# CristianSimion5/vk-raytracing-engine

Measured on AMD Instinct MI355X. Metric: Mrays/s, higher is better.
Workload: dtype f32

## Files before the change

include/vkrt.h:

```cpp
#ifndef VKRT_H
#define VKRT_H

#include <stdint.h>
#include "vkrt_host_device.h"

#ifdef __cplusplus
extern "C" {
#endif

#define VKRT_ABI_VERSION 4

enum vkrt_status {
  VKRT_OK = 0,
  VKRT_ERR_INVALID_ARGUMENT = 1,
  VKRT_ERR_NO_DEVICE = 2,
  VKRT_ERR_HIP = 3,
  VKRT_ERR_OUT_OF_MEMORY = 4,
  VKRT_ERR_NOT_BUILT = 5,
  VKRT_ERR_UNSUPPORTED = 6
};

typedef struct vkrt_scene vkrt_scene;

typedef struct vkrt_prim_mesh {
// ... 86 lines not shown
  uint32_t build_flags;
  float    sah_cost;
  float    build_ms;
  uint64_t node_bytes;
  uint64_t triangle_bytes;
  uint32_t reference_count;
  uint32_t reserved;
} vkrt_accel_info;

int         vkrt_abi_version(void);
const char* vkrt_last_error(void);
int         vkrt_device_count(void);

int  vkrt_scene_create(const vkrt_scene_desc* desc, int device, vkrt_scene** out);
void vkrt_scene_destroy(vkrt_scene* scene);

enum vkrt_option {
  VKRT_OPT_MODE            = 1,
  VKRT_OPT_BVH_LAYOUT      = 2,
  VKRT_OPT_WF_SUBFRAMES    = 3,
  VKRT_OPT_WF_TRAV_BLOCK   = 4,
  VKRT_OPT_WF_SHARE        = 5,
  VKRT_OPT_TRI_THRESHOLD   = 6,
  VKRT_OPT_WF_SHARE_PERIOD = 7,
  VKRT_OPT_WF_SHARE_FLAGS  = 8,
  VKRT_OPT_GBUFFER_MIPS    = 9,
  VKRT_OPT_WATERTIGHT      = 10,
  VKRT_OPT_SKIP_DEAD_SHADOW_RAYS = 11,
  VKRT_OPT_ANYHIT_DISSOLVE = 12,
  VKRT_OPT_WF_FRAMES_IN_FLIGHT = 13,
  VKRT_OPT_SPLIT_BUDGET    = 14,
  VKRT_OPT_LAST            = 14,
  VKRT_OPT_WF_SAMPLE_SYNC  = 15,
  VKRT_INFO_ANYHIT_ORDER   = 100,
  VKRT_INFO_SPLIT_BUDGET   = 101
};
int vkrt_scene_set_option(vkrt_scene* scene, int option, int value);
int vkrt_scene_get_option(const vkrt_scene* scene, int option, int* value);

int vkrt_accel_build(vkrt_scene* scene, uint32_t build_flags, void* hip_stream);
int vkrt_accel_get_info(const vkrt_scene* scene, vkrt_accel_info* out);

int vkrt_scene_update_nodes(vkrt_scene* scene, uint32_t first, uint32_t count, const vkrt_node* nodes, void* hip_stream);
int vkrt_accel_refit(vkrt_scene* scene, void* hip_stream);

enum vkrt_memory { VKRT_MEMORY_HOST = 0, VKRT_MEMORY_DEVICE = 1 };
typedef struct vkrt_vertex_update {
  uint32_t struct_size;
  uint32_t first, count;
  uint32_t memory;
  const float* positions;
  const float* normals;
  const float* tangents;
  const float* texcoords0;
} vkrt_vertex_update;
int vkrt_scene_update_vertices(vkrt_scene* scene, const vkrt_vertex_update* update, void* hip_stream);

typedef struct vkrt_ray {
  float origin[3];    float tmin;
  float direction[3]; float tmax;
} vkrt_ray;
typedef struct vkrt_hit {
  float   t, u, v;
  int32_t instance;
  int32_t primitive;
  int32_t prim_mesh;
// ... 146 lines not shown
```

vk-raytracing-engine_amd/abi.py:

```python
import ctypes as C

c_f = C.c_float
c_i = C.c_int32
c_u = C.c_uint32
c_u64 = C.c_uint64


class Mat4(C.Structure):
    _fields_ = [("m", c_f * 16)]


class GlobalUniforms(C.Structure):
    _fields_ = [("viewProj", Mat4), ("viewInverse", Mat4), ("projInverse", Mat4)]


class PushConstantRay(C.Structure):
    _fields_ = [
        ("clearColor", c_f * 4),
        ("frame", c_i),
        ("lightsCount", c_i),
        ("samples", c_i),
        ("depth", c_i),
        ("useShadows", c_i),
        ("useAO", c_i),
# ... 170 lines not shown
                ("tangents", C.c_void_p), ("texcoords0", C.c_void_p)]


assert C.sizeof(VertexUpdate) == 48
assert C.sizeof(Ray) == 32
assert C.sizeof(Hit) == 32
assert C.sizeof(Surface) == 128
assert C.sizeof(InstanceVisibility) == 4
assert C.sizeof(QueryOpts) == 16

assert C.sizeof(GlobalUniforms) == 192
assert C.sizeof(PushConstantRay) == 44
assert C.sizeof(PrimMeshInfo) == 12
assert C.sizeof(GltfPBRMaterial) == 52
assert C.sizeof(GltfLight) == 32
assert C.sizeof(PrimMesh) == 20
assert C.sizeof(Node) == 68

VKRT_OK, VKRT_ERR_INVALID_ARGUMENT, VKRT_ERR_NO_DEVICE, VKRT_ERR_HIP, VKRT_ERR_OUT_OF_MEMORY, VKRT_ERR_NOT_BUILT, VKRT_ERR_UNSUPPORTED = range(7)
VKRT_BUILD_LBVH_GPU = 0x1
VKRT_BUILD_SAH_HOST = 0x2
VKRT_BUILD_PLOC_GPU = 0x4
VKRT_TRACE_SEED_INDEX_ROW_MAJOR = 0x1
VKRT_TRACE_COUNT_TRAVERSAL = 0x2
VKRT_TRACE_TIME_KERNELS = 0x4
VKRT_TRACE_SAME_SEED_EVERY_FRAME = 0x8
VKRT_ABI_VERSION = 4
VKRT_OPT_MODE, VKRT_OPT_BVH_LAYOUT, VKRT_OPT_WF_SUBFRAMES, VKRT_OPT_WF_TRAV_BLOCK = 1, 2, 3, 4
VKRT_OPT_WF_SHARE, VKRT_OPT_TRI_THRESHOLD, VKRT_OPT_WF_SHARE_PERIOD, VKRT_OPT_WF_SHARE_FLAGS = 5, 6, 7, 8
VKRT_OPT_GBUFFER_MIPS = 9
VKRT_OPT_WATERTIGHT, VKRT_OPT_SKIP_DEAD_SHADOW_RAYS, VKRT_OPT_ANYHIT_DISSOLVE = 10, 11, 12
VKRT_OPT_WF_FRAMES_IN_FLIGHT, VKRT_OPT_SPLIT_BUDGET = 13, 14
VKRT_OPT_WF_SAMPLE_SYNC = 15
VKRT_INFO_ANYHIT_ORDER = 100
VKRT_INFO_SPLIT_BUDGET = 101
VKRT_INSTANCE_FACING_CULL_DISABLE, VKRT_INSTANCE_FLIP_FACING = 0x1, 0x2
VKRT_RAY_OPAQUE, VKRT_RAY_CULL_BACK_FACING, VKRT_RAY_CULL_FRONT_FACING = 0x1, 0x10, 0x20
VKRT_MEMORY_HOST, VKRT_MEMORY_DEVICE = 0, 1
VKRT_SURFACE_GEOMETRY, VKRT_SURFACE_MATERIAL = 0x1, 0x2
VKRT_MULTIHIT_MAX = 16

VKRT_SYMBOLS = [
    "vkrt_abi_version",
    "vkrt_last_error",
    "vkrt_device_count",
    "vkrt_scene_create",
    "vkrt_scene_destroy",
    "vkrt_scene_set_option",
    "vkrt_scene_get_option",
    "vkrt_reserve",
    "vkrt_reserve_frames",
    "vkrt_accel_build",
    "vkrt_accel_get_info",
    "vkrt_scene_update_nodes",
    "vkrt_accel_refit",
    "vkrt_scene_update_vertices",
    "vkrt_intersect",
    "vkrt_occluded",
    "vkrt_scene_set_instance_visibility",
    "vkrt_scene_get_instance_visibility",
    "vkrt_intersect_ex",
    "vkrt_occluded_ex",
    "vkrt_intersect_multi",
    "vkrt_closest_point",
    "vkrt_hit_surface",
    "vkrt_shard_rows",
# ... 122 lines not shown
```

vk-raytracing-engine_amd/csrc/device_scene.h:

```cpp
#pragma once
#include <hip/hip_runtime.h>
#include <stdint.h>
#include "../../include/vkrt_host_device.h"
#include "device_math.h"

struct DevInstance
{
  float o2w[12];
  float w2o[9];
  int32_t primMesh;
  uint32_t vis;
  int32_t pad;
};
static_assert(sizeof(DevInstance) == 96, "DevInstance");
#define VKRT_VIS_CULL_DISABLE 0x100u
#define VKRT_VIS_FLIP 0x200u
#define VKRT_VIS_MIRRORED 0x10000u

#define VKRT_VERTEX_QUADS 3
#define VKRT_VERTEX_BYTES 48u
struct DevTexRef
{
  uint32_t offset;
  uint32_t wh;
// ... 66 lines not shown
  unsigned long long* faults;
};
struct DevQueryScene : DevScene
{
  const uint2* nodeMasks;
  uint32_t cullMask;
  uint32_t rayFlags;
};
struct DevSurfaceScene : DevScene
{
  const uint4* primMeshes;
  uint32_t instanceCount;
};

#define VKRT_TRAV_FAULT(sc) atomicAdd((sc).faults, 1ull)

#ifndef VKRT_W8_MAX_POSTPONED
#define VKRT_W8_MAX_POSTPONED 8
#endif
#ifndef VKRT_W8_POSTPONE_ROOM
#define VKRT_W8_POSTPONE_ROOM 0
#endif

#define VKRT_COUNTER_SLOTS 64
struct DevCounters
{
  unsigned long long v[VKRT_COUNTER_SLOTS][VKRT_COUNTER_STRIDE];
};

#define VKRT_TRACE_PUBLIC_FLAGS 0xFu
#define VKRT_FLAG_SKIP_DEAD_SHADOW 0x100u
#define VKRT_FLAG_STORE_STAGED 0x200u
#define VKRT_FLAG_SAMPLE_SYNC 0x400u

struct TraceParams
{
  DevScene sc;
  PushConstantRay pc;
  float viewInverse[16];
  float projInverse[16];
  uint32_t seed;
  uint32_t flags;
  uint32_t fullW, fullH;
  uint32_t stripRows, shardCount, shardIndex;
  uint32_t localRows;
  uint32_t tilesX, tileCount;
  uint32_t tileFirst;
  float* image;
  unsigned int* workCounter;
  DevCounters* counters;
};

struct WfBuffers
{
  unsigned* ctrl;
  float4* planes;
  float4* stage;
  uint32_t capacity;
  uint32_t groups;
  float4* sampleState;
};
```

vk-raytracing-engine_amd/csrc/kernels.h:

```cpp
#pragma once
#include <hip/hip_runtime.h>
#include "device_scene.h"

hipError_t vkrt_launch_pathtrace(const TraceParams& P, unsigned gridBlocks, bool count, hipStream_t stream);
int        vkrt_pathtrace_block_size();
hipError_t vkrt_pathtrace_occupancy(size_t ldsBytes, int* blocksPerCU);
hipError_t vkrt_launch_trace_rays(const DevScene& sc, unsigned n, const float* o, const float* d, float tmin, float tmax, int anyHit,
                                  float* t, float* u, float* v, int* gid, hipStream_t stream);
hipError_t vkrt_launch_eval_math(int op, unsigned n, const float* a, const float* b, float* out, hipStream_t stream);

hipError_t vkrt_launch_query(const DevQueryScene& sc, const float4* rays, uint64_t n, uint32_t seed, bool filter, bool opaque, float4* hits, int* occ,
                             hipStream_t stream);
hipError_t vkrt_launch_query_multi(const DevQueryScene& sc, const float4* rays, uint64_t n, uint32_t seed, bool filter, bool opaque, uint32_t maxHits,
                                   float4* hits, int* counts, hipStream_t stream);
hipError_t vkrt_launch_closest_point(const DevQueryScene& sc, const float4* queries, uint64_t n, bool filter, float4* hits, unsigned long long* work,
                                     hipStream_t stream);
hipError_t vkrt_launch_node_masks(const DevScene& sc, uint32_t nodeCount, uint32_t instCount, uint32_t sweeps, uint2* masks, hipStream_t stream);
hipError_t vkrt_launch_hit_surface(const DevSurfaceScene& sc, const float4* hits, uint32_t n, bool material, float4* out, hipStream_t stream);

struct WfTiming
{
  hipEvent_t* events;
  int capacity;
  int used;
};
#define VKRT_WF_MAX_LANES 8
struct WfAsync
{
  hipStream_t streams[VKRT_WF_MAX_LANES];
  hipEvent_t fork, join[VKRT_WF_MAX_LANES];
  int count;
  hipEvent_t* pool;
  int poolSize;
};
inline int vkrt_wf_pool_events(int frames, int lanes) { return frames * lanes; }
size_t     vkrt_wf_state_bytes(uint32_t pathCapacity, int groups);
void       vkrt_wf_carve(void* base, uint32_t pathCapacity, int groups, WfBuffers* B);
struct WfOptions
{
  int subframes;
  int travBlock;
  int inFlight;
};
hipError_t vkrt_launch_wavefront(const TraceParams& P, const WfBuffers& B, const WfOptions& opt, int frames, uint32_t seedStep, bool count,
                                 hipStream_t stream, WfTiming* timing, const WfAsync* async);
void       vkrt_wf_launch_traverse(const TraceParams& P, const WfBuffers& B, int r, unsigned travBlock, bool count, dim3 tg, size_t tlds,
                                   hipStream_t stream);

struct HybridGi
{
  float4* color;
  float4* position;
  float4* normal;
  float2* rough;
  float4* accum;
  float4* nrdRadHitD;
  float* nrdViewZ;
};
hipError_t vkrt_launch_gbuffer(const TraceParams& P, const float clearColor[4], int lightsCount, const HybridGi& G, float* nrdNormRough,
                               const float* viewMatrix, hipStream_t stream);
hipError_t vkrt_launch_hybrid(const TraceParams& P, const HybridGi& G, uint2* giLater, hipStream_t stream);
hipError_t vkrt_launch_hybrid_gi(const TraceParams& P, const WfBuffers& B, const HybridGi& G, unsigned travBlock, hipStream_t stream);
uint2* vkrt_wf_hybrid_tmp(const WfBuffers& B);
hipError_t vkrt_launch_post(int rtMode, int viewAccumulated, int useGI, unsigned n, const float* mainImg, const float* rtImg, float* out,
                            hipStream_t stream);

struct DenoiseParams
{
  uint32_t W, H;
  const float4* color;
  const float4* position;
  const float4* normal;
  const float2* rough;
  const float* viewZ;
  const float4* radHitD;
  const float4* histColor;
  const float4* geomPrev;
  float4* geomCur;
  const float4* momPrev;
  float4* momCur;
// ... 25 lines not shown
```

vk-raytracing-engine_amd/csrc/vkrt_api.cpp:

```cpp
#include <hip/hip_runtime.h>

#include <algorithm>
#include <chrono>
#include <cmath>
#include <cstdarg>
#include <cstdio>
#include <cstdlib>
#include <cstring>
#include <initializer_list>
#include <string>
#include <vector>

#include "../../include/vkrt.h"
#include "bvh_host.h"
#include "dev_buffer.h"
#include "device_scene.h"
#include "kernels.h"
#include "wide_node.h"

#define VKRT_TRI_THRESHOLD_DEFAULT 32
#define VKRT_WF_SHARE_DEFAULT 16
#define VKRT_WF_SHARE_FLAGS_DEFAULT 25
#define VKRT_WF_FRAMES_IN_FLIGHT_DEFAULT 3
#define VKRT_SPLIT_BUDGET_DEFAULT -1
#define VKRT_WF_SAMPLE_SYNC_DEFAULT 1
#include "lbvh.h"
#include "refit.h"
#include "vertex_update.h"

namespace {

thread_local std::string g_lastError;

int fail(int code, const char* fmt, ...)
{
  char buf[512];
  va_list ap;
  va_start(ap, fmt);
  vsnprintf(buf, sizeof buf, fmt, ap);
  va_end(ap);
  g_lastError = buf;
  return code;
}

#define HIP_TRY(expr)                                                      \
  do                                                                       \
  {                                                                        \
    std::string m_;                                                        \
    if(const int rc_ = vkrt::hip_status((expr), #expr, m_); rc_ != VKRT_OK) \
      return fail(rc_, "%s", m_.c_str());                                  \
  } while(0)

}

struct vkrt_scene
{
  int device = 0;
  int cuCount = 256;
  std::vector<float> positions;
  std::vector<uint32_t> indices;
  std::vector<vkrt_prim_mesh> primMeshes;
  std::vector<vkrt_node> nodes;
  uint32_t lightCount = 0, materialCount = 0;
  std::vector<float> materialAlpha;
  std::vector<void*> allocs;
  DevScene dev{};
  vkrt::TreeBuffers accel;
  bool built = false;
  vkrt_accel_info info{};
  unsigned int* workCounter = nullptr;
  DevCounters* counters = nullptr;
  hipEvent_t evStart = nullptr, evStop = nullptr;
  bool timed = false;
  void* wfMem = nullptr;
  WfBuffers wf{};
  WfAsync wfAsync{};
  std::vector<hipEvent_t> wfEvents;
  WfTiming wfTiming{};
  bool wfTimed = false;
  int splitResolved = 0;
  int wfTimingRounds = 0;
  std::vector<hipEvent_t> wfPool;
  int opt[VKRT_OPT_WF_SAMPLE_SYNC + 1] = {0, 1, 1, 3, 64, VKRT_WF_SHARE_DEFAULT, VKRT_TRI_THRESHOLD_DEFAULT, 0, VKRT_WF_SHARE_FLAGS_DEFAULT, 1, 0, 0, 0,
                                          VKRT_WF_FRAMES_IN_FLIGHT_DEFAULT, VKRT_SPLIT_BUDGET_DEFAULT, VKRT_WF_SAMPLE_SYNC_DEFAULT};
  bool hasLargeTriangles = false;
  bool wavefront = true;
  bool stale = false;
  bool refitted = false;
  vkrt::RefitScratch refit;
  bool positionsOnDevice = false;
  vkrt::DevBuf vertexStage;
  size_t vertexStageBytes = 0;
  std::vector<vkrt_instance_visibility> vis;
  uint64_t masksPresent[4] = {0, 0, 0, 0};
  vkrt::DevBuf nodeMasks;
  const uint4* surfacePrimMeshes = nullptr;
};

namespace {

template <typename T>
int upload(vkrt_scene* s, const T* src, size_t count, const T** dst)
{
  void* p = nullptr;
  const size_t bytes = std::max<size_t>(count * sizeof(T), 16);
  HIP_TRY(hipMalloc(&p, bytes));
  s->allocs.push_back(p);
  if(count)
    HIP_TRY(hipMemcpy(p, src, count * sizeof(T), hipMemcpyHostToDevice));
  *dst = (const T*)p;
  return VKRT_OK;
}

int checkTransform(const vkrt_node& n, uint32_t i)
{
  for(int k = 0; k < 16; k++)
    if(!std::isfinite(n.worldMatrix[k]))
// ... 65 lines not shown
      const float flx = floorf(fu), fly = floorf(fv), ax = fu - flx, ay = fv - fly;
      auto cl = [](int v, int n) { return v < 0 ? 0 : (v >= n ? n - 1 : v); };
      const int x0 = cl((int)flx, (int)sw), x1 = cl((int)flx + 1, (int)sw), y0 = cl((int)fly, (int)sh), y1 = cl((int)fly + 1, (int)sh);
      const uint32_t p[4] = {src[(size_t)y0 * sw + x0], src[(size_t)y0 * sw + x1], src[(size_t)y1 * sw + x0], src[(size_t)y1 * sw + x1]};
      uint32_t out = 0;
      for(int c = 0; c < 4; c++)
      {
        const uint32_t base = (srgb && c < 3) ? 0u : 256u;
        const float t00 = lut512[base + ((p[0] >> (8 * c)) & 255u)], t10 = lut512[base + ((p[1] >> (8 * c)) & 255u)];
        const float t01 = lut512[base + ((p[2] >> (8 * c)) & 255u)], t11 = lut512[base + ((p[3] >> (8 * c)) & 255u)];
        float v = (t00 * (1.0f - ax) + t10 * ax) * (1.0f - ay) + (t01 * (1.0f - ax) + t11 * ax) * ay;
        if(srgb && c < 3) v = srgbEncode(v);
        v = v < 0.0f ? 0.0f : (v > 1.0f ? 1.0f : v);
        out |= (uint32_t)(v * 255.0f + 0.5f) << (8 * c);
      }
      dst[(size_t)y * dw + x] = out;
    }
}

bool useWavefront(const vkrt_scene* s) { return s->opt[VKRT_OPT_MODE] == 1; }

int clampOption(int option, int v)
{
  switch(option)
  {
    case VKRT_OPT_MODE: case VKRT_OPT_BVH_LAYOUT: return v ? 1 : 0;
    case VKRT_OPT_WF_SUBFRAMES: case VKRT_OPT_WF_FRAMES_IN_FLIGHT: return std::max(1, std::min(VKRT_WF_MAX_LANES, v));
    case VKRT_OPT_SPLIT_BUDGET: return std::max(-1, std::min(100, v));
    case VKRT_OPT_WF_TRAV_BLOCK: return v == 256 ? 256 : v == 128 ? 128 : 64;
    case VKRT_OPT_WF_SHARE: return std::max(0, std::min(64, v));
    case VKRT_OPT_TRI_THRESHOLD: return std::max(0, std::min(65, v));
    case VKRT_OPT_WF_SHARE_PERIOD: return std::max(0, std::min(255, v));
    case VKRT_OPT_WF_SHARE_FLAGS: return v & 31;
    case VKRT_OPT_GBUFFER_MIPS: case VKRT_OPT_WATERTIGHT: case VKRT_OPT_SKIP_DEAD_SHADOW_RAYS: case VKRT_OPT_ANYHIT_DISSOLVE: case VKRT_OPT_WF_SAMPLE_SYNC: return v ? 1 : 0;
  }
  return v;
}

void optionsFromEnvironment(vkrt_scene* s)
{
  const char* e;
  if((e = getenv("VKRT_MODE")) && !strcmp(e, "mega")) s->opt[VKRT_OPT_MODE] = 0;
  if((e = getenv("VKRT_BVH")) && !strcmp(e, "bvh2")) s->opt[VKRT_OPT_BVH_LAYOUT] = 0;
  const struct { const char* name; int option; } ints[] = {{"VKRT_WF_SUBFRAMES", VKRT_OPT_WF_SUBFRAMES}, {"VKRT_WF_TRAV_BLOCK", VKRT_OPT_WF_TRAV_BLOCK},
                                                          {"VKRT_WF_SHARE", VKRT_OPT_WF_SHARE}, {"VKRT_TRI_THRESHOLD", VKRT_OPT_TRI_THRESHOLD},
                                                          {"VKRT_WF_SHARE_PERIOD", VKRT_OPT_WF_SHARE_PERIOD}, {"VKRT_WF_SHARE_FLAGS", VKRT_OPT_WF_SHARE_FLAGS},
                                                          {"VKRT_GBUFFER_MIPS", VKRT_OPT_GBUFFER_MIPS}, {"VKRT_WATERTIGHT", VKRT_OPT_WATERTIGHT},
                                                          {"VKRT_SKIP_DEAD_SHADOW_RAYS", VKRT_OPT_SKIP_DEAD_SHADOW_RAYS},
                                                          {"VKRT_ANYHIT_DISSOLVE", VKRT_OPT_ANYHIT_DISSOLVE}, {"VKRT_WF_FRAMES_IN_FLIGHT", VKRT_OPT_WF_FRAMES_IN_FLIGHT},
                                                          {"VKRT_SPLIT_BUDGET", VKRT_OPT_SPLIT_BUDGET}, {"VKRT_WF_SAMPLE_SYNC", VKRT_OPT_WF_SAMPLE_SYNC}};
  for(const auto& k : ints)
    if((e = getenv(k.name)))
      s->opt[k.option] = clampOption(k.option, atoi(e));
}

void freeAccel(vkrt_scene* s)
{
  s->accel = vkrt::TreeBuffers{};
  s->nodeMasks = vkrt::DevBuf{};
  s->built = false;
  s->refit = vkrt::RefitScratch{};
  s->refitted = false;
  s->stale = false;
}

constexpr vkrt_instance_visibility kDefaultVisibility = {0xFF, VKRT_INSTANCE_FACING_CULL_DISABLE, 0};

void makeInstance(const vkrt_node& node, const vkrt_instance_visibility& vis, DevInstance& in)
{
  memset(&in, 0, sizeof in);
  for(int r = 0; r < 3; r++)
    for(int c = 0; c < 4; c++)
      in.o2w[r * 4 + c] = node.worldMatrix[c * 4 + r];
  vkrt::invert3x3_rows(in.o2w, in.w2o);
  in.primMesh = node.primMesh;
  const float* m = in.o2w;
  const double det = (double)m[0] * ((double)m[5] * m[10] - (double)m[6] * m[9]) - (double)m[1] * ((double)m[4] * m[10] - (double)m[6] * m[8]) +
                     (double)m[2] * ((double)m[4] * m[9] - (double)m[5] * m[8]);
  in.vis = (uint32_t)vis.mask | ((uint32_t)vis.flags << 8) | (det < 0.0 ? VKRT_VIS_MIRRORED : 0u);
}

void noteMasks(vkrt_scene* s)
{
// ... 463 lines not shown
  *out = s;
  return VKRT_OK;
}

void vkrt_scene_destroy(vkrt_scene* s)
{
  if(!s)
    return;
  (void)hipSetDevice(s->device);
  freeAccel(s);
  for(void* p : s->allocs)
    (void)hipFree(p);
  if(s->wfMem) (void)hipFree(s->wfMem);
  if(s->wfAsync.count)
  {
    (void)hipEventDestroy(s->wfAsync.fork);
    for(int j = 0; j < s->wfAsync.count; j++)
    {
      (void)hipStreamDestroy(s->wfAsync.streams[j]);
      (void)hipEventDestroy(s->wfAsync.join[j]);
    }
  }
  for(hipEvent_t e : s->wfEvents) (void)hipEventDestroy(e);
  for(hipEvent_t e : s->wfPool) (void)hipEventDestroy(e);
  if(s->evStart) (void)hipEventDestroy(s->evStart);
  if(s->evStop) (void)hipEventDestroy(s->evStop);
  delete s;
}

int vkrt_scene_set_option(vkrt_scene* s, int option, int value)
{
  if(!s)
    return fail(VKRT_ERR_INVALID_ARGUMENT, "scene is NULL");
  if(option < VKRT_OPT_MODE || option > VKRT_OPT_WF_SAMPLE_SYNC)
    return fail(VKRT_ERR_INVALID_ARGUMENT, "unknown option %d", option);
  if(clampOption(option, value) != value)
    return fail(VKRT_ERR_INVALID_ARGUMENT, "option %d: value %d out of range", option, value);
  s->opt[option] = value;
  return VKRT_OK;
}

int vkrt_scene_get_option(const vkrt_scene* s, int option, int* value)
{
  if(!s || !value)
    return fail(VKRT_ERR_INVALID_ARGUMENT, "NULL argument");
  if(option == VKRT_INFO_ANYHIT_ORDER)
  {
    *value = s->built ? (int)(s->dev.shareFlags & 6u) : 0;
    return VKRT_OK;
  }
  if(option == VKRT_INFO_SPLIT_BUDGET)
  {
    *value = s->built ? s->splitResolved : 0;
    return VKRT_OK;
  }
  if(option < VKRT_OPT_MODE || option > VKRT_OPT_WF_SAMPLE_SYNC)
    return fail(VKRT_ERR_INVALID_ARGUMENT, "unknown option %d", option);
  *value = s->opt[option];
  return VKRT_OK;
}

int vkrt_reserve(vkrt_scene* s, const vkrt_shard* shard, void* hip_stream)
{
  if(!s)
    return fail(VKRT_ERR_INVALID_ARGUMENT, "NULL argument");
  return vkrt_reserve_frames(s, shard, (uint32_t)std::max(1, s->opt[VKRT_OPT_WF_FRAMES_IN_FLIGHT]), hip_stream);
}

int vkrt_reserve_frames(vkrt_scene* s, const vkrt_shard* shard, uint32_t frames_per_call, void* hip_stream)
{
  if(!s || !shard)
    return fail(VKRT_ERR_INVALID_ARGUMENT, "NULL argument");
  if(frames_per_call == 0)
    return fail(VKRT_ERR_INVALID_ARGUMENT, "frames_per_call is 0");
  int rc = checkShard(shard);
  if(rc == VKRT_OK)
    rc = setDevice(s);
  if(rc != VKRT_OK)
    return rc;
  const uint64_t tiles = (uint64_t)((shard->full_width + 7) / 8) * ((vkrt_shard_rows(shard) + 7) / 8);
  if(tiles * 64 >= 0xFFFFFFFFull)
    return fail(VKRT_ERR_UNSUPPORTED, "launch too large");
  const bool wavefront = s->built ? s->wavefront : useWavefront(s);
  if(tiles == 0 || !wavefront)
    return VKRT_OK;
  int rc2 = ensureWorkingSet(s, (uint32_t)tiles * 64u, framesInFlight(s, (int)std::min<uint32_t>(frames_per_call, VKRT_FRAMES_PER_BATCH)), (hipStream_t)hip_stream);
  if(rc2 == VKRT_OK)
    rc2 = ensureEventPool(s, (int)std::min<uint32_t>(frames_per_call, VKRT_FRAMES_PER_BATCH));
  return rc2;
// ... 557 lines not shown
    return fail(VKRT_ERR_INVALID_ARGUMENT, "n_frames %u out of range", n_frames);
  if(!image && vkrt_shard_rows(shard) != 0u)
    return fail(VKRT_ERR_INVALID_ARGUMENT, "NULL image");
  int rc = checkBuilt(s, "vkrt_pathtrace");
  if(rc == VKRT_OK)
    rc = checkShard(shard);
  if(rc != VKRT_OK)
    return rc;
  if(pc->lightsCount < 0 || (uint32_t)pc->lightsCount > s->lightCount)
    return fail(VKRT_ERR_INVALID_ARGUMENT, "PushConstantRay.lightsCount %d outside [0,%u]", pc->lightsCount, s->lightCount);
  if(pc->samples < 0 || pc->depth < 0 || pc->depth > 99)
    return fail(VKRT_ERR_INVALID_ARGUMENT, "samples/depth out of range");
  if((rc = setDevice(s)) != VKRT_OK)
    return rc;
  hipStream_t stream = (hipStream_t)hip_stream;
  TraceParams P;
  if((rc = launchParams(s, pc, cam, opts, shard, P)) != VKRT_OK)
    return rc;
  if(P.localRows == 0)
    return VKRT_OK;
  if(s->opt[VKRT_OPT_SKIP_DEAD_SHADOW_RAYS])
    P.flags |= VKRT_FLAG_SKIP_DEAD_SHADOW;
  P.image = image;
  P.workCounter = s->workCounter;

  const bool count = (P.flags & VKRT_TRACE_COUNT_TRAVERSAL) != 0;
  if(s->wavefront)
  {
    if(P.fullW > 65535u || P.localRows > 65535u || pc->samples > 65535)
      return fail(VKRT_ERR_UNSUPPORTED, "wavefront mode packs pixel coordinates / sample index in 16 bits");
    const uint32_t seedStep = (P.flags & VKRT_TRACE_SAME_SEED_EVERY_FRAME) ? 0u : 1u;
    if(s->opt[VKRT_OPT_WF_SAMPLE_SYNC])
      P.flags |= VKRT_FLAG_SAMPLE_SYNC;
    if((rc = ensureWorkingSet(s, P.tileCount * 64u, framesInFlight(s, (int)n_frames), stream)) != VKRT_OK)
      return rc;
    if((rc = ensureEventPool(s, (int)std::min<uint32_t>(n_frames, VKRT_FRAMES_PER_BATCH))) != VKRT_OK)
      return rc;
    WfTiming* timing = nullptr;
    if(P.flags & VKRT_TRACE_TIME_KERNELS)
    {
      const size_t wantEv = (size_t)2 * (2 * (size_t)pc->samples * pc->depth) * std::min<uint32_t>(n_frames, 8u);
      while(s->wfEvents.size() < wantEv && s->wfEvents.size() < 8192)
      {
        hipEvent_t e;
        HIP_TRY(hipEventCreate(&e));
        s->wfEvents.push_back(e);
      }
      s->wfTiming.events = s->wfEvents.data();
      s->wfTiming.capacity = (int)s->wfEvents.size();
      timing = &s->wfTiming;
    }
    s->wfTimed = timing != nullptr;
    s->wfTimingRounds = (pc->samples > 0 && pc->depth > 0) ? pc->samples * (pc->depth + 1) : 0;
    HIP_TRY(hipEventRecord(s->evStart, stream));
    WfOptions wo;
    wo.subframes = s->opt[VKRT_OPT_WF_SUBFRAMES];
    wo.travBlock = travBlock(s);
    wo.inFlight = framesInFlight(s, (int)n_frames);
    if(timing)
      timing->used = 0;
    for(uint32_t first = 0; first < n_frames; first += VKRT_FRAMES_PER_BATCH)
    {
      TraceParams Pb = P;
      Pb.pc.frame = P.pc.frame + (int)first;
      Pb.seed = P.seed + first * seedStep;
      HIP_TRY(vkrt_launch_wavefront(Pb, s->wf, wo, (int)std::min<uint32_t>(VKRT_FRAMES_PER_BATCH, n_frames - first), seedStep, count, stream, timing, &s->wfAsync));
// ... 678 lines not shown
```

vk-raytracing-engine_amd/csrc/wavefront.hip:

```cpp
#include <hip/hip_runtime.h>
#include <algorithm>
#include <cstdlib>
#include <cstring>

#include "device_math.h"
#include "device_scene.h"
#include "kernels.h"
#include "rgen.h"
#include "hybrid_gi.h"
#include "shade.h"
#include "traverse.h"
#include "traverse_wide.h"
#include "traverse_share.h"

#define WF_BLOCK 256
#define VKRT_FLAG_COUNT_WORK 2u

#include "wf_streams.h"

VKRT_DEV unsigned packFlags(const LaneState& L)
{
  return (L.prd.depth & 0xffu) | (((unsigned)L.smpl & 0xffffu) << 8) | ((L.prd.isSpecular ? 1u : 0u) << 25);
}

// ... 118 lines not shown
  LaneState L;
  uint32_t x, y, lrow;
  if(pixelOfWork(P, w, P.tileFirst, x, y, lrow))
  {
    const float4 st = wfLoad(B.sampleState + pixelSlot(P, x, lrow));
    bindPixel(P, L, x, lrow);
    L.prd.seed = __float_as_uint(st.w);
    L.hitValues = mk3(st.x, st.y, st.z);
    L.smpl = smpl;
    startSample(P, L);
    alive = true;
  }
  __shared__ unsigned wsum[WF_TYPES * (WF_BLOCK / 64 + 1)];
  const unsigned slot = claimSlots(B, round & 1, alive ? WF_C : -1, lane, wsum);
  if(alive)
    storeClosest(B, round & 1, slot, L);
}

VKRT_DEV bool advanceSegmentHybrid(const TraceParams& P, const HybridGi& G, LaneState& L, bool shadowHit, f3 contrib, f3 nextWeight, float lightDist)
{
  L.stage = 0;
  if(giSegmentStep(P.pc, L.prd, L.curWeight, L.hitValue, L.hitValues.x, shadowHit, contrib, nextWeight, lightDist))
    return true;
  hybridStorePixel(P, G, (size_t)L.lrow * P.fullW + L.px, true, L.hitValue, L.hitValues.x, L.hitValues.y);
  return false;
}

struct ShadeLds
{
  float lut[512];
  unsigned wsum[WF_TYPES * (WF_BLOCK / 64 + 1)];
};

template <bool PAIR, bool HYBRID>
VKRT_DEV void shadeHitBlock(const TraceParams& P, const WfBuffers& B, const HybridGi& G, const int par, const unsigned count, const unsigned block, ShadeLds& lds)
{
  const int type = PAIR ? WF_P : WF_C;
  const unsigned lane = lane_id();
  const unsigned qi = block * WF_BLOCK + threadIdx.x;
  ShadeStats st = shadeStatsInit(P.sc, lds.lut);
  unsigned* wsum = lds.wsum;
  int to = -1;
  LaneState L;
  f3 contrib = mk3(0.0f), nextWeight = mk3(0.0f);
  if(qi < count)
  {
    loadCommon(P, B, par, type, qi, L);
    const float4 h = wfLoad(rec(B, par, type, WF_H0, qi)), t4 = wfLoad(rec(B, par, type, WF_H1, qi));
    const float4 rd = wfLoad(rec(B, par, type, PAIR ? WF_R2 : WF_R1, qi));
    L.prd.rayDirection = mk3(rd.x, rd.y, rd.z);
    L.prd.rayOrigin = mk3(0.0f);
    if(PAIR)
    {
      const float4 s3 = wfLoad(rec(B, par, WF_P, WF_S3, qi));
      const bool shadowHit = __float_as_int(h.x) != 0;
      if(HYBRID)
        (void)advanceSegmentHybrid(P, G, L, shadowHit, mk3(s3.x, s3.y, s3.z), L.curWeight, L.prd.depth == 1u ? wfLoad(rec(B, par, WF_P, WF_R1, qi)).w : 0.0f);
      else
        (void)advanceSegment(P, L, shadowHit, mk3(s3.x, s3.y, s3.z), L.curWeight);
    }
    RayHit hit;
    hit.t = h.x; hit.u = h.y; hit.v = h.z; hit.slot = __float_as_int(h.w);
    const uint4 ts = make_uint4(__float_as_uint(t4.x), __float_as_uint(t4.y), __float_as_uint(t4.z), __float_as_uint(t4.w));
    if(hit.slot >= 0)
      closestHitShaderInst(P.sc, P.pc, hit, (uint32_t)hit.slot, ts, L.prd.rayDirection, L.prd, st);
    else
      missShader(P.pc, L.prd);
    segmentTerms(L.prd, L.curWeight, contrib, nextWeight);
    const bool dead = !HYBRID && (P.flags & VKRT_FLAG_SKIP_DEAD_SHADOW) != 0u && contrib.x == 0.0f && contrib.y == 0.0f && contrib.z == 0.0f;
    if(!L.prd.isSpecular && L.prd.depth != 100u && !dead)
      to = (L.prd.depth + 1u < (uint32_t)P.pc.depth) ? WF_P : WF_S;
    else if(HYBRID)
      to = advanceSegmentHybrid(P, G, L, false, contrib, nextWeight, 0.0f) ? WF_C : -1;
    else
      to = finishSegment(P, B, L, false, contrib, nextWeight);
  }
  const unsigned slot = claimSlots(B, par ^ 1, to, lane, wsum);
  if(to == WF_C)
    storeClosest(B, par ^ 1, slot, L);
  else if(to >= 0)
    storeShadow(B, par ^ 1, to, slot, L, contrib, nextWeight);
  if(P.flags & VKRT_FLAG_COUNT_WORK)
  {
// ... 22 lines not shown
      toClosest = advanceSegmentHybrid(P, G, L, shadowHit, mk3(s3.x, s3.y, s3.z), L.curWeight, L.prd.depth == 1u ? wfLoad(rec(B, par, WF_S, WF_R1, qi)).w : 0.0f);
    else
      toClosest = finishSegment(P, B, L, shadowHit, mk3(s3.x, s3.y, s3.z), L.curWeight) == WF_C;
  }
  const unsigned slot = claimSlots(B, par ^ 1, toClosest ? WF_C : -1, lane, wsum);
  if(toClosest)
    storeClosest(B, par ^ 1, slot, L);
}

template <bool HYBRID>
VKRT_DEV void shadeRound(const TraceParams& P, const WfBuffers& B, const HybridGi& G, const int round)
{
  const int par = round & 1;
  const unsigned cC = *countOf(B, par, WF_C), cS = *countOf(B, par, WF_S), cP = *countOf(B, par, WF_P);
  const unsigned nC = (cC + WF_BLOCK - 1) / WF_BLOCK, nP = (cP + WF_BLOCK - 1) / WF_BLOCK, nS = (cS + WF_BLOCK - 1) / WF_BLOCK;
  unsigned blk = blockIdx.x;
  __shared__ ShadeLds lds;
  if(blk < nC)
    shadeHitBlock<false, HYBRID>(P, B, G, par, cC, blk, lds);
  else if((blk -= nC) < nP)
    shadeHitBlock<true, HYBRID>(P, B, G, par, cP, blk, lds);
  else if((blk -= nP) < nS)
    shadeShadowBlock<HYBRID>(P, B, G, par, cS, blk, lds);
}
__global__ __launch_bounds__(WF_BLOCK) void k_wf_shade(const TraceParams P, const WfBuffers B, const int round)
{
  const HybridGi none{};
  shadeRound<false>(P, B, none, round);
}
__global__ __launch_bounds__(WF_BLOCK) void k_wf_shade_hybrid(const TraceParams P, const WfBuffers B, const HybridGi G, const int round)
{
  shadeRound<true>(P, B, G, round);
}

__global__ __launch_bounds__(WF_BLOCK) void k_hy_gi_init(const TraceParams P, const WfBuffers B, const HybridGi G, const uint2* tmp)
{
  const unsigned lane = lane_id();
  const unsigned w = blockIdx.x * blockDim.x + threadIdx.x;
  bool alive = false;
  LaneState L;
  uint32_t x, y, lrow;
  if(pixelOfWork(P, w, P.tileFirst, x, y, lrow))
  {
    const size_t p = (size_t)lrow * P.fullW + x;
    const GbufferPixel g = loadGbufferPixel(G, p);
    const uint2 t = tmp[p];
    const float alpha = __uint_as_float(t.y);
    if(g.shaded)
    {
      bindPixel(P, L, x, lrow);
      L.prd.seed = t.x;
      giFirstRay(P, g, L.prd, L.curWeight);
      L.hitValue = mk3(0.0f);
      L.hitValues = mk3(0.0f, alpha, 0.0f);
      L.smpl = 0;
      L.stage = 0;
      alive = L.prd.depth < (uint32_t)P.pc.depth;
    }
    if(!alive)
      hybridStorePixel(P, G, p, g.shaded, mk3(0.0f), 0.0f, alpha);
  }
  __shared__ unsigned wsum[WF_TYPES * (WF_BLOCK / 64 + 1)];
  const unsigned slot = claimSlots(B, 0, alive ? WF_C : -1, lane, wsum);
  if(alive)
    storeClosest(B, 0, slot, L);
}
// ... 1 lines not shown
__global__ __launch_bounds__(WF_BLOCK) void k_wf_blend(const TraceParams P, const float4* stage)
{
  uint32_t x, y, lrow;
  if(pixelOfWork(P, blockIdx.x * blockDim.x + threadIdx.x, P.tileFirst, x, y, lrow))
  {
    const size_t p = (size_t)lrow * P.fullW + x;
    blendPixel((float4*)P.image + p, stage[p], P.pc.frame);
  }
}

#define WF_CTRL_BYTES (256 * VKRT_WF_MAX_LANES)
size_t vkrt_wf_state_bytes(uint32_t pathCapacity, int groups)
{
  const size_t g = (size_t)std::max(groups, 1);
  return g * pathCapacity * 2 * WF_SLOTS * sizeof(float4) + (g > 1 ? g * pathCapacity * sizeof(float4) : 0) + g * pathCapacity * sizeof(float4) +
         WF_CTRL_BYTES;
}

void vkrt_wf_carve(void* base, uint32_t pathCapacity, int groups, WfBuffers* B)
{
  const size_t g = (size_t)std::max(groups, 1);
  char* p = (char*)base;
  B->ctrl = (unsigned*)p;
  p += WF_CTRL_BYTES;
  B->planes = (float4*)p;
  p += g * pathCapacity * 2 * WF_SLOTS * sizeof(float4);
  B->stage = g > 1 ? (float4*)p : nullptr;
  p += g > 1 ? g * pathCapacity * sizeof(float4) : 0;
  B->sampleState = (float4*)p;
  B->capacity = pathCapacity;
  B->groups = (uint32_t)g;
}

static hipError_t subframeBegin(const TraceParams& P, const WfBuffers& B, hipStream_t stream)
{
  const unsigned work = P.tileCount * 64u;
  const hipError_t e = hipMemsetAsync(B.ctrl, 0, 64, stream);
  if(e != hipSuccess)
    return e;
  hipLaunchKernelGGL(k_wf_init, dim3((work + WF_BLOCK - 1) / WF_BLOCK), dim3(WF_BLOCK), 0, stream, P, B);
  return hipSuccess;
}
static int subframeRounds(const TraceParams& P) { return (P.pc.samples <= 0 || P.pc.depth <= 0) ? 0 : P.pc.samples * (P.pc.depth + 1); }
static void launchTraverse(const TraceParams& P, const WfBuffers& B, int r, unsigned travBlock, bool count, hipStream_t stream)
{
  const unsigned work = P.tileCount * 64u, tb = (travBlock == 256u || travBlock == 128u) ? travBlock : 64u;
  vkrt_wf_launch_traverse(P, B, r, tb, count, dim3(2 * ((work + tb - 1) / tb) + 4), (size_t)P.sc.stackCap * tb * sizeof(int), stream);
}
static void subframeRound(const TraceParams& P, const WfBuffers& B, int r, unsigned travBlock, bool count, hipStream_t stream, WfTiming* timing)
{
  const unsigned work = P.tileCount * 64u;
  const bool timed = timing && timing->events && 2 * (timing->used + 1) <= timing->capacity;
  if(timed)
    (void)hipEventRecord(timing->events[2 * timing->used], stream);
  launchTraverse(P, B, r, travBlock, count, stream);
  if(timed)
  {
    (void)hipEventRecord(timing->events[2 * timing->used + 1], stream);
    timing->used++;
  }
  hipLaunchKernelGGL(k_wf_shade, dim3((work + WF_BLOCK - 1) / WF_BLOCK + 3), dim3(WF_BLOCK), 0, stream, P, B, r);
}

static bool sampleSync(const TraceParams& P) { return (P.flags & VKRT_FLAG_SAMPLE_SYNC) != 0u; }
static int subframeSteps(const TraceParams& P) { return subframeRounds(P) + ((sampleSync(P) && subframeRounds(P) > 0) ? P.pc.samples - 1 : 0); }
static void subframeStep(const TraceParams& P, const WfBuffers& B, int step, unsigned travBlock, bool count, hipStream_t stream, WfTiming* timing)
{
  if(!sampleSync(P))
    return subframeRound(P, B, step, travBlock, count, stream, timing);
  const int perSample = P.pc.depth + 2;
  const int s = (step + 1) / perSample, k = (step + 1) % perSample;
  if(k != 0)
    return subframeRound(P, B, s * (P.pc.depth + 1) + k - 1, travBlock, count, stream, timing);
  const unsigned work = P.tileCount * 64u;
  hipLaunchKernelGGL(k_wf_sample_init, dim3((work + WF_BLOCK - 1) / WF_BLOCK), dim3(WF_BLOCK), 0, stream, P, B, s * (P.pc.depth + 1), s);
}

static TraceParams frameParams(const TraceParams& P, int k, uint32_t seedStep)
{
  TraceParams Q = P;
  Q.pc.frame = P.pc.frame + k;
  Q.seed = P.seed + (uint32_t)k * seedStep;
  return Q;
}

static int balancedInFlight(int frames, int want)
{
  want = std::max(1, std::min(want, frames));
  const int turns = (frames + want - 1) / want;
  return (frames + turns - 1) / turns;
}

hipError_t vkrt_launch_wavefront(const TraceParams& P, const WfBuffers& B, const WfOptions& opt, int frames, uint32_t seedStep, bool count,
                                 hipStream_t stream, WfTiming* timing, const WfAsync* async)
{
  const unsigned travBlock = (unsigned)opt.travBlock;
  const int steps = subframeSteps(P);
  frames = std::max(frames, 1);
  int F = (timing || !async || steps == 0) ? 1 : std::min(balancedInFlight(frames, opt.inFlight), (int)B.groups);
  F = std::max(1, std::min(F, async ? std::min(VKRT_WF_MAX_LANES, async->count) : 1));
// ... 145 lines not shown
```

vk-raytracing-engine_amd/csrc/wf_traverse.hip:

```cpp
#include <hip/hip_runtime.h>

#include "device_math.h"
#include "device_scene.h"
#include "kernels.h"
#include "traverse.h"
#include "traverse_wide.h"
#include "traverse_share.h"
#include "wf_streams.h"

enum { WF_K_CLOSEST_C = 0, WF_K_CLOSEST_P = 1, WF_K_SHADOW_S = 2, WF_K_SHADOW_P = 3 };

VKRT_DEV void storeHit(const TraceParams& P, const WfBuffers& B, int par, int kind, unsigned qi, const RayHit& hit)
{
  if(kind == WF_K_SHADOW_S)
    wfStore(rec(B, par, WF_S, WF_H0, qi), make_float4(0.0f, 0.0f, 0.0f, __int_as_float(hit.slot >= 0 ? 0 : -1)));
  else if(kind == WF_K_SHADOW_P)
    ((float*)rec(B, par, WF_P, WF_H0, qi))[0] = __int_as_float(hit.slot >= 0 ? 1 : 0);
  else
  {
    const int type = kind == WF_K_CLOSEST_C ? WF_C : WF_P;
    int inst = -1;
    if(hit.slot >= 0)
    {
      const uint4 ts = P.sc.triShade[hit.slot];
      inst = __float_as_int(P.sc.tris[hit.slot * VKRT_TRI_QUADS + 2].z);
      wfStore(rec(B, par, type, WF_H1, qi), make_float4(__uint_as_float(ts.x), __uint_as_float(ts.y), __uint_as_float(ts.z), __uint_as_float(ts.w)));
    }
    float* h = (float*)rec(B, par, type, WF_H0, qi);
    if(type == WF_C)
      wfStore(rec(B, par, WF_C, WF_H0, qi), make_float4(hit.t, hit.u, hit.v, __int_as_float(inst)));
    else
    {
      h[1] = hit.u; h[2] = hit.v; h[3] = __int_as_float(inst);
    }
  }
}

// ... 32 lines not shown
    r1 = wfLoad(rec(B, par, type, kind == WF_K_CLOSEST_P ? WF_R2 : WF_R1, qi));
    if(kind == WF_K_CLOSEST_P)
      r0.w = 10000.0f;
  }
  uint32_t raySeed = 0u;
  if((TM & VKRT_TM_DISSOLVE) && valid)
    raySeed = __float_as_uint(wfLoad(rec(B, par, type, WF_S0, qi)).w);
  TravCount tc;
  __shared__ int shareLds[VKRT_SHARE_LDS_WORDS];
  RayHit hit;
  if(WIDE && TB == 64 && P.sc.shareMinIdle != 0u && P.sc.triThreshold != 0u)
  {
    uint2* stk = ((uint2*)lds_stack) + threadIdx.x;
    if(anyHit)
      traverse_wide8_share<COUNT, true, TM>(P.sc, valid, mk3(r0.x, r0.y, r0.z), mk3(r1.x, r1.y, r1.z), 0.001f, r0.w, stk, shareRes(shareLds), hit, tc, raySeed);
    else
      traverse_wide8_share<COUNT, false, TM>(P.sc, valid, mk3(r0.x, r0.y, r0.z), mk3(r1.x, r1.y, r1.z), 0.001f, r0.w, stk, shareRes(shareLds), hit, tc, raySeed);
    if(valid)
      storeHit(P, B, par, kind, qi, hit);
  }
  else if(valid)
  {
    traverse_any<COUNT, WIDE, TM>(P.sc, mk3(r0.x, r0.y, r0.z), mk3(r1.x, r1.y, r1.z), 0.001f, r0.w, anyHit, lds_stack, (int)threadIdx.x, TB, hit, tc, raySeed);
    storeHit(P, B, par, kind, qi, hit);
  }
  if(COUNT)
  {
    __shared__ unsigned long long red[VKRT_COUNTER_STRIDE * (TB / 64)];
    const unsigned vals[10] = {0, 0, 0, 0, 0, 0, tc.nodes, tc.tris, tc.waveNodeSteps, tc.waveTriSteps};
    blockAddCounters(&P.counters->v[blockIdx.x % VKRT_COUNTER_SLOTS][0], vals, 10, red);
  }
}

void vkrt_wf_launch_traverse(const TraceParams& P, const WfBuffers& B, int r, unsigned travBlock, bool count, dim3 tg, size_t tlds, hipStream_t stream)
{
  const bool wide = P.sc.layout == 1u;
  const dim3 tb(travBlock);
#define VKRT_TRAV_LAUNCH(C, W, TB, TM) hipLaunchKernelGGL((k_wf_traverse<C, W, TB, TM>), tg, tb, tlds, stream, P, B, r)
#define VKRT_TRAV_MODES(TB, TM)                                                                                                        \
  do {                                                                                                                                 \
    if(wide) { if(count) VKRT_TRAV_LAUNCH(true, true, TB, TM); else VKRT_TRAV_LAUNCH(false, true, TB, TM); }                           \
    else { if(count) VKRT_TRAV_LAUNCH(true, false, TB, TM); else VKRT_TRAV_LAUNCH(false, false, TB, TM); }                             \
  } while(0)
#define VKRT_TRAV_64(TM) VKRT_TRAV_MODES(64, TM)
  if(travBlock == 64)
  {
    VKRT_FRAME_TM_SWITCH(frame_tri_mode(P.sc, false), VKRT_TM_DISSOLVE, VKRT_TRAV_64)
  }
  else if(travBlock == 128)
    VKRT_TRAV_MODES(128, 0);
  else
    VKRT_TRAV_MODES(256, 0);
#undef VKRT_TRAV_64
#undef VKRT_TRAV_MODES
#undef VKRT_TRAV_LAUNCH
}
```

Baseline: 5311.

## Generate camera rays inside a dedicated traverse kernel for primary wavefront rounds

Adds a camera-round path that regenerates primary rays per pixel directly in a specialized traverse kernel and a camera-specific shade kernel. It skips the init kernel and the separate per-sample sync steps, and it avoids writing and reading primary ray records through global memory. The path is enabled by default when sample sync, the wide layout, 64-thread traversal and sharing are active. In exchange, ray generation work is repeated in both the traverse and shade kernels, and the code adds more kernel variants.

```diff
diff --git a/include/vkrt.h b/include/vkrt.h
--- a/include/vkrt.h
+++ b/include/vkrt.h
@@ -142,6 +142,7 @@
   VKRT_OPT_SPLIT_BUDGET    = 14,
   VKRT_OPT_LAST            = 14,
   VKRT_OPT_WF_SAMPLE_SYNC  = 15,
+  VKRT_OPT_WF_CAMERA_ROUNDS = 16,
   VKRT_INFO_ANYHIT_ORDER   = 100,
   VKRT_INFO_SPLIT_BUDGET   = 101
 };
diff --git a/vk-raytracing-engine_amd/abi.py b/vk-raytracing-engine_amd/abi.py
--- a/vk-raytracing-engine_amd/abi.py
+++ b/vk-raytracing-engine_amd/abi.py
@@ -226,6 +226,7 @@
 VKRT_OPT_WATERTIGHT, VKRT_OPT_SKIP_DEAD_SHADOW_RAYS, VKRT_OPT_ANYHIT_DISSOLVE = 10, 11, 12
 VKRT_OPT_WF_FRAMES_IN_FLIGHT, VKRT_OPT_SPLIT_BUDGET = 13, 14
 VKRT_OPT_WF_SAMPLE_SYNC = 15
+VKRT_OPT_WF_CAMERA_ROUNDS = 16
 VKRT_INFO_ANYHIT_ORDER = 100
 VKRT_INFO_SPLIT_BUDGET = 101
 VKRT_INSTANCE_FACING_CULL_DISABLE, VKRT_INSTANCE_FLIP_FACING = 0x1, 0x2
diff --git a/vk-raytracing-engine_amd/csrc/device_scene.h b/vk-raytracing-engine_amd/csrc/device_scene.h
--- a/vk-raytracing-engine_amd/csrc/device_scene.h
+++ b/vk-raytracing-engine_amd/csrc/device_scene.h
@@ -122,6 +122,7 @@
 #define VKRT_FLAG_SKIP_DEAD_SHADOW 0x100u
 #define VKRT_FLAG_STORE_STAGED 0x200u
 #define VKRT_FLAG_SAMPLE_SYNC 0x400u
+#define VKRT_FLAG_CAMERA_ROUNDS 0x800u
 
 struct TraceParams
 {
diff --git a/vk-raytracing-engine_amd/csrc/kernels.h b/vk-raytracing-engine_amd/csrc/kernels.h
--- a/vk-raytracing-engine_amd/csrc/kernels.h
+++ b/vk-raytracing-engine_amd/csrc/kernels.h
@@ -46,6 +46,7 @@
                                  hipStream_t stream, WfTiming* timing, const WfAsync* async);
 void       vkrt_wf_launch_traverse(const TraceParams& P, const WfBuffers& B, int r, unsigned travBlock, bool count, dim3 tg, size_t tlds,
                                    hipStream_t stream);
+void       vkrt_wf_launch_traverse_camera(const TraceParams& P, const WfBuffers& B, int r, int smpl, bool count, size_t tlds, hipStream_t stream);
 
 struct HybridGi
 {
diff --git a/vk-raytracing-engine_amd/csrc/vkrt_api.cpp b/vk-raytracing-engine_amd/csrc/vkrt_api.cpp
--- a/vk-raytracing-engine_amd/csrc/vkrt_api.cpp
+++ b/vk-raytracing-engine_amd/csrc/vkrt_api.cpp
@@ -24,6 +24,7 @@
 #define VKRT_WF_FRAMES_IN_FLIGHT_DEFAULT 3
 #define VKRT_SPLIT_BUDGET_DEFAULT -1
 #define VKRT_WF_SAMPLE_SYNC_DEFAULT 1
+#define VKRT_WF_CAMERA_ROUNDS_DEFAULT 1
 #include "lbvh.h"
 #include "refit.h"
 #include "vertex_update.h"
@@ -81,8 +82,8 @@
   int splitResolved = 0;
   int wfTimingRounds = 0;
   std::vector<hipEvent_t> wfPool;
-  int opt[VKRT_OPT_WF_SAMPLE_SYNC + 1] = {0, 1, 1, 3, 64, VKRT_WF_SHARE_DEFAULT, VKRT_TRI_THRESHOLD_DEFAULT, 0, VKRT_WF_SHARE_FLAGS_DEFAULT, 1, 0, 0, 0,
-                                          VKRT_WF_FRAMES_IN_FLIGHT_DEFAULT, VKRT_SPLIT_BUDGET_DEFAULT, VKRT_WF_SAMPLE_SYNC_DEFAULT};
+  int opt[VKRT_OPT_WF_CAMERA_ROUNDS + 1] = {0, 1, 1, 3, 64, VKRT_WF_SHARE_DEFAULT, VKRT_TRI_THRESHOLD_DEFAULT, 0, VKRT_WF_SHARE_FLAGS_DEFAULT, 1, 0, 0, 0,
+                                            VKRT_WF_FRAMES_IN_FLIGHT_DEFAULT, VKRT_SPLIT_BUDGET_DEFAULT, VKRT_WF_SAMPLE_SYNC_DEFAULT, VKRT_WF_CAMERA_ROUNDS_DEFAULT};
   bool hasLargeTriangles = false;
   bool wavefront = true;
   bool stale = false;
@@ -214,7 +215,8 @@
     case VKRT_OPT_TRI_THRESHOLD: return std::max(0, std::min(65, v));
     case VKRT_OPT_WF_SHARE_PERIOD: return std::max(0, std::min(255, v));
     case VKRT_OPT_WF_SHARE_FLAGS: return v & 31;
-    case VKRT_OPT_GBUFFER_MIPS: case VKRT_OPT_WATERTIGHT: case VKRT_OPT_SKIP_DEAD_SHADOW_RAYS: case VKRT_OPT_ANYHIT_DISSOLVE: case VKRT_OPT_WF_SAMPLE_SYNC: return v ? 1 : 0;
+    case VKRT_OPT_GBUFFER_MIPS: case VKRT_OPT_WATERTIGHT: case VKRT_OPT_SKIP_DEAD_SHADOW_RAYS: case VKRT_OPT_ANYHIT_DISSOLVE: case VKRT_OPT_WF_SAMPLE_SYNC:
+    case VKRT_OPT_WF_CAMERA_ROUNDS: return v ? 1 : 0;
   }
   return v;
 }
@@ -230,7 +232,8 @@
                                                           {"VKRT_GBUFFER_MIPS", VKRT_OPT_GBUFFER_MIPS}, {"VKRT_WATERTIGHT", VKRT_OPT_WATERTIGHT},
                                                           {"VKRT_SKIP_DEAD_SHADOW_RAYS", VKRT_OPT_SKIP_DEAD_SHADOW_RAYS},
                                                           {"VKRT_ANYHIT_DISSOLVE", VKRT_OPT_ANYHIT_DISSOLVE}, {"VKRT_WF_FRAMES_IN_FLIGHT", VKRT_OPT_WF_FRAMES_IN_FLIGHT},
-                                                          {"VKRT_SPLIT_BUDGET", VKRT_OPT_SPLIT_BUDGET}, {"VKRT_WF_SAMPLE_SYNC", VKRT_OPT_WF_SAMPLE_SYNC}};
+                                                          {"VKRT_SPLIT_BUDGET", VKRT_OPT_SPLIT_BUDGET}, {"VKRT_WF_SAMPLE_SYNC", VKRT_OPT_WF_SAMPLE_SYNC},
+                                                          {"VKRT_WF_CAMERA_ROUNDS", VKRT_OPT_WF_CAMERA_ROUNDS}};
   for(const auto& k : ints)
     if((e = getenv(k.name)))
       s->opt[k.option] = clampOption(k.option, atoi(e));
@@ -760,7 +763,7 @@
 {
   if(!s)
     return fail(VKRT_ERR_INVALID_ARGUMENT, "scene is NULL");
-  if(option < VKRT_OPT_MODE || option > VKRT_OPT_WF_SAMPLE_SYNC)
+  if(option < VKRT_OPT_MODE || option > VKRT_OPT_WF_CAMERA_ROUNDS)
     return fail(VKRT_ERR_INVALID_ARGUMENT, "unknown option %d", option);
   if(clampOption(option, value) != value)
     return fail(VKRT_ERR_INVALID_ARGUMENT, "option %d: value %d out of range", option, value);
@@ -782,7 +785,7 @@
     *value = s->built ? s->splitResolved : 0;
     return VKRT_OK;
   }
-  if(option < VKRT_OPT_MODE || option > VKRT_OPT_WF_SAMPLE_SYNC)
+  if(option < VKRT_OPT_MODE || option > VKRT_OPT_WF_CAMERA_ROUNDS)
     return fail(VKRT_ERR_INVALID_ARGUMENT, "unknown option %d", option);
   *value = s->opt[option];
   return VKRT_OK;
@@ -1406,6 +1409,9 @@
     const uint32_t seedStep = (P.flags & VKRT_TRACE_SAME_SEED_EVERY_FRAME) ? 0u : 1u;
     if(s->opt[VKRT_OPT_WF_SAMPLE_SYNC])
       P.flags |= VKRT_FLAG_SAMPLE_SYNC;
+    if(s->opt[VKRT_OPT_WF_CAMERA_ROUNDS] && (P.flags & VKRT_FLAG_SAMPLE_SYNC) && s->dev.layout == 1u && travBlock(s) == 64 && s->dev.shareMinIdle != 0u &&
+       s->dev.triThreshold != 0u)
+      P.flags |= VKRT_FLAG_CAMERA_ROUNDS;
     if((rc = ensureWorkingSet(s, P.tileCount * 64u, framesInFlight(s, (int)n_frames), stream)) != VKRT_OK)
       return rc;
     if((rc = ensureEventPool(s, (int)std::min<uint32_t>(n_frames, VKRT_FRAMES_PER_BATCH))) != VKRT_OK)
diff --git a/vk-raytracing-engine_amd/csrc/wavefront.hip b/vk-raytracing-engine_amd/csrc/wavefront.hip
--- a/vk-raytracing-engine_amd/csrc/wavefront.hip
+++ b/vk-raytracing-engine_amd/csrc/wavefront.hip
@@ -174,8 +174,9 @@
   unsigned wsum[WF_TYPES * (WF_BLOCK / 64 + 1)];
 };
 
-template <bool PAIR, bool HYBRID>
-VKRT_DEV void shadeHitBlock(const TraceParams& P, const WfBuffers& B, const HybridGi& G, const int par, const unsigned count, const unsigned block, ShadeLds& lds)
+template <bool PAIR, bool HYBRID, bool CAMERA = false>
+VKRT_DEV void shadeHitBlock(const TraceParams& P, const WfBuffers& B, const HybridGi& G, const int par, const unsigned count, const unsigned block, ShadeLds& lds,
+                            const int smpl = 0)
 {
   const int type = PAIR ? WF_P : WF_C;
   const unsigned lane = lane_id();
@@ -185,12 +186,34 @@
   int to = -1;
   LaneState L;
   f3 contrib = mk3(0.0f), nextWeight = mk3(0.0f);
-  if(qi < count)
-  {
-    loadCommon(P, B, par, type, qi, L);
+  uint32_t x = 0, y = 0, lrow = 0;
+  if(CAMERA ? pixelOfWork(P, qi, P.tileFirst, x, y, lrow) : qi < count)
+  {
+    if(CAMERA)
+    {
+      bindPixel(P, L, x, lrow);
+      if(smpl == 0)
+      {
+        L.prd.seed = pixelSeed(P, x, y);
+        L.hitValues = mk3(0.0f);
+      }
+      else
+      {
+        const float4 s = wfLoad(B.sampleState + pixelSlot(P, x, lrow));
+        L.prd.seed = __float_as_uint(s.w);
+        L.hitValues = mk3(s.x, s.y, s.z);
+      }
+      L.smpl = smpl;
+      startSample(P, L);
+    }
+    else
+      loadCommon(P, B, par, type, qi, L);
     const float4 h = wfLoad(rec(B, par, type, WF_H0, qi)), t4 = wfLoad(rec(B, par, type, WF_H1, qi));
-    const float4 rd = wfLoad(rec(B, par, type, PAIR ? WF_R2 : WF_R1, qi));
-    L.prd.rayDirection = mk3(rd.x, rd.y, rd.z);
+    if(!CAMERA)
+    {
+      const float4 rd = wfLoad(rec(B, par, type, PAIR ? WF_R2 : WF_R1, qi));
+      L.prd.rayDirection = mk3(rd.x, rd.y, rd.z);
+    }
     L.prd.rayOrigin = mk3(0.0f);
     if(PAIR)
     {
@@ -279,6 +302,12 @@
 {
   shadeRound<true>(P, B, G, round);
 }
+__global__ __launch_bounds__(WF_BLOCK) void k_wf_shade_camera(const TraceParams P, const WfBuffers B, const int round, const int smpl)
+{
+  const HybridGi none{};
+  __shared__ ShadeLds lds;
+  shadeHitBlock<false, false, true>(P, B, none, round & 1, 0u, blockIdx.x, lds, smpl);
+}
 
 __global__ __launch_bounds__(WF_BLOCK) void k_hy_gi_init(const TraceParams P, const WfBuffers B, const HybridGi G, const uint2* tmp)
 {
@@ -346,40 +375,54 @@
   B->groups = (uint32_t)g;
 }
 
+static int subframeRounds(const TraceParams& P) { return (P.pc.samples <= 0 || P.pc.depth <= 0) ? 0 : P.pc.samples * (P.pc.depth + 1); }
+static bool cameraRounds(const TraceParams& P) { return (P.flags & VKRT_FLAG_CAMERA_ROUNDS) != 0u && subframeRounds(P) > 0; }
 static hipError_t subframeBegin(const TraceParams& P, const WfBuffers& B, hipStream_t stream)
 {
   const unsigned work = P.tileCount * 64u;
   const hipError_t e = hipMemsetAsync(B.ctrl, 0, 64, stream);
   if(e != hipSuccess)
     return e;
-  hipLaunchKernelGGL(k_wf_init, dim3((work + WF_BLOCK - 1) / WF_BLOCK), dim3(WF_BLOCK), 0, stream, P, B);
+  if(!cameraRounds(P))
+    hipLaunchKernelGGL(k_wf_init, dim3((work + WF_BLOCK - 1) / WF_BLOCK), dim3(WF_BLOCK), 0, stream, P, B);
   return hipSuccess;
 }
-static int subframeRounds(const TraceParams& P) { return (P.pc.samples <= 0 || P.pc.depth <= 0) ? 0 : P.pc.samples * (P.pc.depth + 1); }
 static void launchTraverse(const TraceParams& P, const WfBuffers& B, int r, unsigned travBlock, bool count, hipStream_t stream)
 {
   const unsigned work = P.tileCount * 64u, tb = (travBlock == 256u || travBlock == 128u) ? travBlock : 64u;
   vkrt_wf_launch_traverse(P, B, r, tb, count, dim3(2 * ((work + tb - 1) / tb) + 4), (size_t)P.sc.stackCap * tb * sizeof(int), stream);
 }
-static void subframeRound(const TraceParams& P, const WfBuffers& B, int r, unsigned travBlock, bool count, hipStream_t stream, WfTiming* timing)
+static void subframeRound(const TraceParams& P, const WfBuffers& B, int r, unsigned travBlock, bool count, hipStream_t stream, WfTiming* timing,
+                          int cameraSample = -1)
 {
   const unsigned work = P.tileCount * 64u;
   const bool timed = timing && timing->events && 2 * (timing->used + 1) <= timing->capacity;
   if(timed)
     (void)hipEventRecord(timing->events[2 * timing->used], stream);
-  launchTraverse(P, B, r, travBlock, count, stream);
+  if(cameraSample >= 0)
+    vkrt_wf_launch_traverse_camera(P, B, r, cameraSample, count, (size_t)P.sc.stackCap * 64u * sizeof(int), stream);
+  else
+    launchTraverse(P, B, r, travBlock, count, stream);
   if(timed)
   {
     (void)hipEventRecord(timing->events[2 * timing->used + 1], stream);
     timing->used++;
   }
-  hipLaunchKernelGGL(k_wf_shade, dim3((work + WF_BLOCK - 1) / WF_BLOCK + 3), dim3(WF_BLOCK), 0, stream, P, B, r);
+  if(cameraSample >= 0)
+    hipLaunchKernelGGL(k_wf_shade_camera, dim3((work + WF_BLOCK - 1) / WF_BLOCK), dim3(WF_BLOCK), 0, stream, P, B, r, cameraSample);
+  else
+    hipLaunchKernelGGL(k_wf_shade, dim3((work + WF_BLOCK - 1) / WF_BLOCK + 3), dim3(WF_BLOCK), 0, stream, P, B, r);
 }
 
 static bool sampleSync(const TraceParams& P) { return (P.flags & VKRT_FLAG_SAMPLE_SYNC) != 0u; }
-static int subframeSteps(const TraceParams& P) { return subframeRounds(P) + ((sampleSync(P) && subframeRounds(P) > 0) ? P.pc.samples - 1 : 0); }
+static int subframeSteps(const TraceParams& P)
+{
+  return subframeRounds(P) + ((sampleSync(P) && !cameraRounds(P) && subframeRounds(P) > 0) ? P.pc.samples - 1 : 0);
+}
 static void subframeStep(const TraceParams& P, const WfBuffers& B, int step, unsigned travBlock, bool count, hipStream_t stream, WfTiming* timing)
 {
+  if(cameraRounds(P))
+    return subframeRound(P, B, step, travBlock, count, stream, timing, step % (P.pc.depth + 1) == 0 ? step / (P.pc.depth + 1) : -1);
   if(!sampleSync(P))
     return subframeRound(P, B, step, travBlock, count, stream, timing);
   const int perSample = P.pc.depth + 2;
diff --git a/vk-raytracing-engine_amd/csrc/wf_traverse.hip b/vk-raytracing-engine_amd/csrc/wf_traverse.hip
--- a/vk-raytracing-engine_amd/csrc/wf_traverse.hip
+++ b/vk-raytracing-engine_amd/csrc/wf_traverse.hip
@@ -3,6 +3,7 @@
 #include "device_math.h"
 #include "device_scene.h"
 #include "kernels.h"
+#include "rgen.h"
 #include "traverse.h"
 #include "traverse_wide.h"
 #include "traverse_share.h"
@@ -101,6 +102,51 @@
   }
 }
 
+template <bool COUNT, int TM>
+__global__ __launch_bounds__(64)
+__attribute__((amdgpu_waves_per_eu(TM != 0 ? 5 : 1)))
+void k_wf_traverse_camera(const TraceParams P, const WfBuffers B, const int round, const int smpl)
+{
+  extern __shared__ int lds_stack[];
+  const int par = round & 1;
+  if(blockIdx.x == 0 && threadIdx.x == 0)
+    for(int t = 0; t < WF_TYPES; t++) *countOf(B, par ^ 1, t) = 0u;
+  const unsigned w = blockIdx.x * 64u + threadIdx.x;
+  uint32_t x = 0, y = 0, lrow = 0;
+  const bool valid = pixelOfWork(P, w, P.tileFirst, x, y, lrow);
+  f3 o = mk3(0.0f), d = mk3(1.0f, 0.0f, 0.0f);
+  uint32_t raySeed = 0u;
+  if(valid)
+  {
+    LaneState L;
+    bindPixel(P, L, x, lrow);
+    L.prd.seed = smpl == 0 ? pixelSeed(P, x, y) : __float_as_uint(((const float*)(B.sampleState + pixelSlot(P, x, lrow)))[3]);
+    L.smpl = smpl;
+    startSample(P, L);
+    o = L.prd.rayOrigin; d = L.prd.rayDirection;
+    raySeed = L.prd.seed;
+  }
+  const unsigned nValid = (unsigned)__popcll(__ballot(valid));
+  if(threadIdx.x == 0 && nValid)
+  {
+    atomicAdd(&P.counters->v[blockIdx.x % VKRT_COUNTER_SLOTS][0], (unsigned long long)nValid);
+    if(smpl == 0) atomicAdd(&P.counters->v[blockIdx.x % VKRT_COUNTER_SLOTS][5], (unsigned long long)nValid);
+  }
+  TravCount tc;
+  __shared__ int shareLds[VKRT_SHARE_LDS_WORDS];
+  RayHit hit;
+  uint2* stk = ((uint2*)lds_stack) + threadIdx.x;
+  traverse_wide8_share<COUNT, false, TM>(P.sc, valid, o, d, 0.001f, 10000.0f, stk, shareRes(shareLds), hit, tc, raySeed);
+  if(valid)
+    storeHit(P, B, par, WF_K_CLOSEST_C, w, hit);
+  if(COUNT)
+  {
+    __shared__ unsigned long long red[VKRT_COUNTER_STRIDE];
+    const unsigned vals[10] = {0, 0, 0, 0, 0, 0, tc.nodes, tc.tris, tc.waveNodeSteps, tc.waveTriSteps};
+    blockAddCounters(&P.counters->v[blockIdx.x % VKRT_COUNTER_SLOTS][0], vals, 10, red);
+  }
+}
+
 void vkrt_wf_launch_traverse(const TraceParams& P, const WfBuffers& B, int r, unsigned travBlock, bool count, dim3 tg, size_t tlds, hipStream_t stream)
 {
   const bool wide = P.sc.layout == 1u;
@@ -124,3 +170,14 @@
 #undef VKRT_TRAV_MODES
 #undef VKRT_TRAV_LAUNCH
 }
+
+void vkrt_wf_launch_traverse_camera(const TraceParams& P, const WfBuffers& B, int r, int smpl, bool count, size_t tlds, hipStream_t stream)
+{
+#define VKRT_TRAV_CAMERA(TM)                                                                                                           \
+  do {                                                                                                                                 \
+    if(count) hipLaunchKernelGGL((k_wf_traverse_camera<true, TM>), dim3(P.tileCount), dim3(64), tlds, stream, P, B, r, smpl);          \
+    else hipLaunchKernelGGL((k_wf_traverse_camera<false, TM>), dim3(P.tileCount), dim3(64), tlds, stream, P, B, r, smpl);              \
+  } while(0)
+  VKRT_FRAME_TM_SWITCH(frame_tri_mode(P.sc, false), VKRT_TM_DISSOLVE, VKRT_TRAV_CAMERA)
+#undef VKRT_TRAV_CAMERA
+}
```

Result: faster. 5399, median of 6 (+1.6%).
